# serval/kaboodle

Hardware: AMD Instinct MI355X
Metric: simulated peer-rounds/sec (whole node) + rounds to fingerprint convergence (higher is better)
Workload: dtype u8

## Files before the change

### kaboodle_amd/csrc/kb_round.h

```cpp
#pragma once
#include "kb_common.h"

namespace kb {

__global__ void k_rebase(Dev d, int32_t r) {
  const size_t total = (size_t)(d.hi - d.lo) * d.W / 16;
  const uint32_t wpr = d.W / 16;
  const int32_t E = epoch_base(r - 1);
  uint4* p = reinterpret_cast<uint4*>(d.stamp + (size_t)d.lo * d.W);
  for (size_t k = (size_t)blockIdx.x * blockDim.x + threadIdx.x; k < total; k += (size_t)gridDim.x * blockDim.x) {
    const uint4 v = p[k];
    uint32_t w[4] = {v.x, v.y, v.z, v.w};
    bool any = false;
#pragma unroll
    for (int q = 0; q < 4; ++q) {
      uint32_t x = w[q], y = 0;
#pragma unroll
      for (int t = 0; t < 4; ++t) {
        uint32_t b = (x >> (8 * t)) & 0xFF;
        if (b > ST_ANCIENT) {
          if (d.tst && b <= ST_ANCIENT + EPOCH) {
            const size_t i = d.lo + k / wpr, j = (k % wpr) * 16 + q * 4 + t;
            d.tst[i * d.W + j] = (int32_t)b - EOFF + E;
            atomicMin(d.tlb + i * (d.W >> 10) + (j >> 10), (int32_t)b - EOFF + E);
// ... 863 lines not shown
    if (threadIdx.x < 5) atomicAdd(&d.ctr[ci[threadIdx.x]], (uint32_t)(s_t[threadIdx.x] / 64));
  }
#endif
  __shared__ unsigned long long s_cnt[RP_WAVES][7];
  if (l == 0) {
    s_cnt[wv][0] = w_lost; s_cnt[wv][1] = w_removed; s_cnt[wv][2] = w_resp; s_cnt[wv][3] = w_bytes;
    s_cnt[wv][4] = a3c.x; s_cnt[wv][5] = a3c.y; s_cnt[wv][6] = a3c.z;
    if (!LDSB && w_nodes && pb.nf) path_hit(d, PATH_PHASEB_HBM);
  }
  __syncthreads();
  if (threadIdx.x < 7) {
    unsigned long long t = 0;
    for (uint32_t k = 0; k < wpb; ++k) t += s_cnt[k][threadIdx.x];
    const int idx[7] = {S_BDROP, S_RMFAILED, S_JRESP, S_ROWB, S_A3ROWS, S_A3DEEP, S_A3CHUNKS};
    if (t) slot_add(d, idx[threadIdx.x], t);
  }
}

__global__ __launch_bounds__(256) void k_probe(Dev d, uint32_t np, int32_t r, uint2* out, uint32_t* cnt, uint32_t cap) {
  const uint32_t i = d.lo + blockIdx.x * blockDim.x + threadIdx.x;
  unsigned long long lost_in = 0, sent = 0, lost_out = 0;
  if (i < d.hi && d.alive[i] && d.start_round[i] < r) {
    const bool f = faults(d, r) && d.loss_thr;
    const uint32_t n = d.n[i];
    for (uint32_t e = 0; e < np; ++e) {
      if (f) {
        const U4 w = philox(i, (uint32_t)r, ((uint32_t)P_PROBE << 24) | (e >> 2), 0, d.k0, d.k1);
        const uint32_t u = (e & 3) == 0 ? w.x : (e & 3) == 1 ? w.y : (e & 3) == 2 ? w.z : w.w;
        if (u < d.loss_thr) { lost_in++; continue; }
      }
      const int64_t o = (int64_t)n - 2;
      bool resp = o <= 0;
      if (!resp) {
        int64_t pct = 100 - o * o; if (pct < 1) pct = 1;
        const uint32_t u = philox(i, (uint32_t)r, ((uint32_t)P_RESPOND << 24) | (1u << 23) | e, 0, d.k0, d.k1).x;
        resp = (int64_t)mulhi(u, 100) < pct;
      }
      if (!resp) continue;
      sent++;
      if (f && philox(i, (uint32_t)r, ((uint32_t)P_PROBE << 24) | (1u << 23) | e, 1, d.k0, d.k1).x < d.loss_thr) { lost_out++; continue; }
      const uint32_t k = atomicAdd(cnt, 1u);
      if (k < cap) out[k] = make_uint2(i, e);
      else set_err(d, DERR_OUTBOX);
    }
  }
  const int idx[3] = {S_BDROP, S_PROBERESP, S_LOSS};
  const unsigned long long v[3] = {lost_in, sent, lost_out};
  stat_add_n(d, idx, v);
}

__device__ inline bool newbit(const unsigned long long* nm, uint32_t e) { return (nm[e >> 6] >> (e & 63)) & 1ull; }
__device__ inline uint32_t mix32(uint32_t x) {
  x ^= x >> 16; x *= 0x7feb352du; x ^= x >> 15; x *= 0x846ca68bu; x ^= x >> 16;
  return x;
}
struct Prp { uint32_t n, c, ma, mc, k[4]; };
__device__ inline Prp prp_make(uint32_t n, const U4& key) {
  const uint32_t lg = n <= 1 ? 0u : 32u - __clz(n - 1u);
  const uint32_t b = lg < 2 ? 2u : lg;
  Prp p;
  p.n = n; p.c = b / 2; p.mc = (1u << p.c) - 1u; p.ma = (1u << (b - p.c)) - 1u;
  p.k[0] = key.x; p.k[1] = key.y; p.k[2] = key.z; p.k[3] = key.w;
  return p;
}
__device__ __attribute__((always_inline)) inline uint32_t prp_pass(uint32_t x, const Prp& p) {
  uint32_t L = x >> p.c, R = x & p.mc;
#pragma unroll
  for (int k = 0; k < 4; ++k) { const uint32_t t = R; R = L ^ (mix32(R ^ p.k[k]) & ((k & 1) ? p.mc : p.ma)); L = t; }
  return (L << p.c) | R;
}
__device__ __attribute__((always_inline)) inline uint32_t prp_eval(uint32_t x, const Prp& p) {
  do { x = prp_pass(x, p); } while (x >= p.n);
  return x;
}
__device__ __attribute__((always_inline)) inline uint32_t prp_walk(uint32_t x, uint32_t n, const U4& key) {
  return prp_eval(x, prp_make(n, key));
}
__device__ inline uint32_t bm_rank(const uint32_t* S, const uint32_t* SP, uint32_t id) {
  const uint32_t blk = id >> 8, w = id >> 5;
  uint32_t r = SP[blk];
  for (uint32_t k = blk * 8; k < w; ++k) r += __popc(S[k]);
  return r + __popc(S[w] & ((1u << (id & 31)) - 1u));
}
__device__ __attribute__((always_inline)) inline uint32_t bm_block(const uint32_t* SP, uint32_t nblk, float ratio,
                                                                   uint32_t b, uint32_t* base) {
  uint32_t g = (uint32_t)((float)b * ratio);
  g = g < nblk ? g : nblk - 1;
  const uint32_t l2 = g >= 2 ? g - 2 : 0, h2 = g + 3 < nblk ? g + 3 : nblk;
  uint32_t v[6];
#pragma unroll
  for (int j = 0; j < 6; ++j) v[j] = SP[l2 + j < h2 ? l2 + j : h2];
  if (v[0] <= b && b < v[5]) {
    uint32_t c = 0, bs = v[0];
#pragma unroll
    for (int j = 1; j < 5; ++j) { const bool le = v[j] <= b; c += le; bs = le ? v[j] : bs; }
    *base = bs;
    return l2 + c;
  }
  uint32_t lo = 0, hi = nblk;
  while (hi - lo > 1) { const uint32_t mid = (lo + hi) >> 1; if (SP[mid] <= b) lo = mid; else hi = mid; }
  *base = SP[lo];
  return lo;
}
__device__ __attribute__((always_inline)) inline uint32_t block_pick(const uint4& q0, const uint4& q1, uint32_t blk,
                                                                     uint32_t rem) {
  const uint32_t p0 = __popc(q0.x), p1 = __popc(q0.y), p2 = __popc(q0.z), p3 = __popc(q0.w);
  const uint32_t p4 = __popc(q1.x), p5 = __popc(q1.y), p6 = __popc(q1.z);
  const uint32_t s01 = p0 + p1, s45 = p4 + p5, s03 = s01 + p2 + p3;
  const bool h1 = rem >= s03;
  rem -= h1 ? s03 : 0u;
  const uint32_t sa = h1 ? s45 : s01;
  const bool h2 = rem >= sa;
  rem -= h2 ? sa : 0u;
  const uint32_t pa = h1 ? (h2 ? p6 : p4) : (h2 ? p2 : p0);
  const bool h3 = rem >= pa;
  rem -= h3 ? pa : 0u;
  const uint32_t wi = (h1 ? 4u : 0u) + (h2 ? 2u : 0u) + (h3 ? 1u : 0u);
  const uint32_t xa = h1 ? (h2 ? (h3 ? q1.w : q1.z) : (h3 ? q1.y : q1.x)) : (h2 ? (h3 ? q0.w : q0.z) : (h3 ? q0.y : q0.x));
  return (blk * 8 + wi) * 32 + select_in_word(xa, rem);
}
__device__ inline uint32_t bm_select(const uint32_t* S, const uint32_t* SP, uint32_t nblk, float ratio, uint32_t b) {
  uint32_t base;
  const uint32_t lo = bm_block(SP, nblk, ratio, b, &base);
  const uint4 q0 = *reinterpret_cast<const uint4*>(S + lo * 8), q1 = *reinterpret_cast<const uint4*>(S + lo * 8 + 4);
  return block_pick(q0, q1, lo, b - base);
}
constexpr uint32_t KB_RESP_U = 2;
constexpr int RESP_U = KB_RESP_U;
constexpr int RESP_KMAX = 9;
struct JoinLds {
  const uint32_t *J, *JM;
  __device__ uint32_t min_from(uint32_t u) const { return JM[u]; }
  __device__ uint32_t at(uint32_t f) const { return J[f]; }
};
struct JoinRegs {
  uint32_t j0, j1, jmin;
  __device__ uint32_t min_from(uint32_t) const { return jmin; }
  __device__ uint32_t at(uint32_t f) const { return f < 64 ? rdl(j0, (int)f) : rdl(j1, (int)(f - 64)); }
};
template <class JA>
__device__ __attribute__((always_inline)) inline void sampled_fill(uint32_t* pay, uint32_t k_first, uint32_t stride,
                                                                   uint32_t cap, const Prp& P, const uint32_t* B,
                                                                   const uint32_t* BP, uint32_t NB, float ratio,
                                                                   const JA& J, uint32_t upto, uint32_t nnew) {
  const uint32_t jmin = J.min_from(upto);
  const uint32_t mcount = k_first < cap ? (cap - k_first + stride - 1) / stride : 0u;
  uint32_t y[RESP_KMAX];
#pragma unroll
  for (int q = 0; q < RESP_KMAX; ++q) y[q] = 0;
  if (4ull * P.n >= 3ull * ((uint64_t)(P.ma + 1) << P.c)) {
#pragma unroll
    for (int q = 0; q < RESP_KMAX; ++q) {
      const bool act = (uint32_t)q < mcount;
      if (!__ballot(act)) break;
      uint32_t x = prp_pass(k_first + stride * q, P);
      while (__ballot(act && x >= P.n)) { if (act && x >= P.n) x = prp_pass(x, P); }
      y[q] = x;
    }
  } else {
    uint32_t m = 0, x = k_first;
    while (__ballot(m < mcount)) {
      if (m < mcount) {
        x = prp_pass(x, P);
        if (x < P.n) {
#pragma unroll
          for (int q = 0; q < RESP_KMAX; ++q) if ((uint32_t)q == m) y[q] = x;
          ++m;
          x = k_first + stride * m;
        }
      }
    }
  }
#pragma unroll
  for (int q0 = 0; q0 < RESP_KMAX; q0 += RESP_U) {
    if ((uint32_t)q0 >= mcount) break;
    uint32_t blk[RESP_U], bb[RESP_U];
    uint4 b0[RESP_U], b1[RESP_U];
#pragma unroll
    for (int u = 0; u < RESP_U; ++u) {
      bb[u] = 0;
      blk[u] = q0 + u < RESP_KMAX ? bm_block(BP, NB, ratio, y[q0 + u < RESP_KMAX ? q0 + u : 0], &bb[u]) : 0u;
    }
#pragma unroll
    for (int u = 0; u < RESP_U; ++u) {
      b0[u] = *reinterpret_cast<const uint4*>(B + blk[u] * 8);
      b1[u] = *reinterpret_cast<const uint4*>(B + blk[u] * 8 + 4);
    }
#pragma unroll
    for (int u = 0; u < RESP_U; ++u) {
      const uint32_t q = q0 + u;
      if (q >= RESP_KMAX || q >= mcount) break;
      const uint32_t yq = y[q];
      uint32_t xq = block_pick(b0[u], b1[u], blk[u], yq - bb[u]);
      if (xq >= jmin) {
        uint32_t e = 0;
        while (true) {
          uint32_t c = 0;
          for (uint32_t f = upto; f < nnew; ++f) c += J.at(f) <= xq;
          if (c == e) break;
          e = c;
          xq = bm_select(B, BP, NB, ratio, yq + e);
        }
      }
      pay[k_first + stride * q] = xq;
    }
  }
}
constexpr uint32_t RESP_LDS_W = 131072;
constexpr uint32_t RESP_JCAP = 1024;
__host__ __device__ inline size_t resp_words(uint32_t NW, uint32_t NB) {
  return (2ull * NW + 2ull * (NB + 1) + 2ull * RESP_JCAP + 1 + 3) & ~3ull;
}

__device__ __attribute__((always_inline)) inline uint32_t block_prefix(const uint32_t* X, uint32_t* XP, uint32_t NB, uint32_t* s_red) {
  const uint32_t t = threadIdx.x, T = blockDim.x;
  const uint32_t per = (NB + T - 1) / T;
  uint32_t bc = 0;
  for (uint32_t k = t * per; k < (t + 1) * per && k < NB; ++k) {
    uint32_t c = 0;
    for (uint32_t w = 0; w < 8; ++w) c += __popc(X[k * 8 + w]);
    XP[k] = c; bc += c;
  }
  uint32_t ex = wave_excl(bc);
  const uint32_t wt = wave_sum(bc);
  __syncthreads();
  if (lane() == 0) s_red[t >> 6] = wt;
  __syncthreads();
  for (uint32_t w = 0; w < (t >> 6); ++w) ex += s_red[w];
  uint32_t tot = 0;
  for (uint32_t w = 0; w < T / 64; ++w) tot += s_red[w];
  for (uint32_t k = t * per; k < (t + 1) * per && k < NB; ++k) { const uint32_t c = XP[k]; XP[k] = ex; ex += c; }
  if (t == 0) XP[NB] = tot;
  __syncthreads();
  return tot;
}

constexpr uint32_t RW_JCAP = 128;
__host__ __device__ inline uint32_t rwave_head(uint32_t NB) { return ((NB + 1 > RW_JCAP ? NB + 1 : RW_JCAP) + 3) & ~3u; }
__host__ __device__ inline uint32_t rwave_words(uint32_t NW, uint32_t NB) { return rwave_head(NB) + NW; }
__device__ inline bool resp_by_wave(const Dev& d, uint32_t i, uint32_t nnew, bool on) {
  return on && d.uniform && nnew <= RW_JCAP && d.n[i] - nnew > d.capj;
}
template <bool SG>
__global__ __launch_bounds__(256) __attribute__((amdgpu_waves_per_eu(4))) void k_resp_wave(Dev d, PhaseB pb, const uint32_t* nodes, const uint32_t* nnodes_p,
                                                   OutBuf ob, int32_t r, uint32_t* rest) {
  extern __shared__ __attribute__((aligned(16))) uint32_t rw_lds[];
  const uint32_t NW = d.NWR, NB = d.W / 256;
  const uint32_t wv = threadIdx.x >> 6, l = lane(), nwv = blockDim.x >> 6;
  uint32_t* BP = rw_lds + (size_t)wv * (SG ? rwave_head(NB) : rwave_words(NW, NB));
  uint32_t* Jt = BP;
  uint32_t* S = BP + rwave_head(NB);
  const uint32_t nnodes = *nnodes_p;
  const bool small_lists = pb.JW <= 64 && pb.nj <= 128;
  const uint32_t js0 = small_lists && l < pb.nj ? pb.bjoin[l].sender : 0u;
  const uint32_t js1 = small_lists && l + 64 < pb.nj ? pb.bjoin[l + 64].sender : 0u;
  const uint32_t stride = gridDim.x * nwv;
  uint32_t it = blockIdx.x * nwv + wv;
  uint32_t inext = it < nnodes ? nodes[it] : 0u;
  for (; it < nnodes; it += stride) {
    const uint32_t i = inext;
    const unsigned long long* nm = pb.newmask + (size_t)i * pb.JW;
    const unsigned long long* rm = pb.respmask + (size_t)i * pb.JW;
    const unsigned long long nmv = small_lists && l < pb.JW ? nm[l] : 0ull;
    const unsigned long long rmv = small_lists && l < pb.JW ? rm[l] : 0ull;
    const uint32_t n_i = d.n[i], nbase_i = pb.nbase[i], poff_i = ob.poff[i], ooff_i = ob.off[i];
    inext = it + stride < nnodes ? nodes[it + stride] : 0u;
    const uint32_t* B = bits_of(d, i);
    const uint4* B4 = reinterpret_cast<const uint4*>(B);
    const bool tdbg = (d.dev & 512) != 0;
    const uint64_t tps = tdbg ? wall_clock64() : 0;
    if (!SG) stage16(reinterpret_cast<uint4*>(S), B4, NW / 4, l, 64);
    uint32_t nnew = 0;
    if (small_lists) nnew = wave_sum((uint32_t)__popcll(nmv));
    else for (uint32_t wj = 0; wj < pb.JW; ++wj) nnew += __popcll(nm[wj]);
    if (!(d.uniform && nnew <= RW_JCAP && n_i - nnew > d.capj)) {
      if (l == 0) rest[atomicAdd(&d.ctr[C_RESTN], 1u)] = i;
      wait_lds();
      __builtin_amdgcn_wave_barrier();
      continue;
    }
    if (l == 0) path_hit(d, SG ? PATH_RESP_WAVE_HBM : PATH_RESP_WAVE);
    uint64_t tp0 = tdbg ? wall_clock64() : 0, tp1 = 0, tp2 = 0;
    if (small_lists) {
      const unsigned long long w0 = ((unsigned long long)rdl((uint32_t)(nmv >> 32), 0) << 32) | rdl((uint32_t)nmv, 0);
      const unsigned long long w1 = ((unsigned long long)rdl((uint32_t)(nmv >> 32), 1) << 32) | rdl((uint32_t)nmv, 1);
      if (l < pb.nj && ((w0 >> l) & 1ull)) Jt[__popcll(w0 & ((1ull << l) - 1ull))] = js0;
      if (l + 64 < pb.nj && ((w1 >> l) & 1ull)) Jt[__popcll(w0) + __popcll(w1 & ((1ull << l) - 1ull))] = js1;
    } else {
      for (uint32_t e = l; e < pb.nj; e += 64) {
        if (!newbit(nm, e)) continue;
        uint32_t pos = __popcll(nm[e >> 6] & ((1ull << (e & 63)) - 1ull));
        for (uint32_t w2 = 0; w2 < (e >> 6); ++w2) pos += __popcll(nm[w2]);
        Jt[pos] = pb.bjoin[e].sender;
      }
    }
    wait_lds();
    __builtin_amdgcn_wave_barrier();
    const uint32_t jr0 = l < nnew ? Jt[l] : 0xFFFFFFFFu, jr1 = l + 64 < nnew ? Jt[l + 64] : 0xFFFFFFFFu;
    uint32_t sm0 = jr0, sm1 = jr1;
#pragma unroll
    for (int o = 1; o < 64; o <<= 1) {
      const uint32_t u0 = __shfl_down(sm0, o, 64), u1 = __shfl_down(sm1, o, 64);
      if (l + o < 64) { sm0 = u0 < sm0 ? u0 : sm0; sm1 = u1 < sm1 ? u1 : sm1; }
    }
    {
      const uint32_t m1 = rdl(sm1, 0);
      sm0 = m1 < sm0 ? m1 : sm0;
    }
    wait_lds();
    __builtin_amdgcn_wave_barrier();
    if (tdbg) tp1 = wall_clock64();
    const uint32_t per = (NB + 63) / 64;
    uint32_t bc = 0, last = 0;
    const uint4* S4 = reinterpret_cast<const uint4*>(SG ? B : S);
    for (uint32_t k = l * per; k < (l + 1) * per && k < NB; ++k) {
      const uint4 q0 = S4[2 * k], q1 = S4[2 * k + 1];
      const uint32_t c = __popc(q0.x) + __popc(q0.y) + __popc(q0.z) + __popc(q0.w) + __popc(q1.x) + __popc(q1.y) +
                         __popc(q1.z) + __popc(q1.w);
      BP[k] = c; bc += c;
      if (c) last = k + 1;
    }
    uint32_t ex = wave_excl(bc);
    const uint32_t nB = wave_sum(bc);
    const uint32_t nbu = wave_max(last);
    const float ratio = nB ? (float)nbu / (float)nB : 0.0f;
    for (uint32_t k = l * per; k < (l + 1) * per && k < NB; ++k) { const uint32_t c = BP[k]; BP[k] = ex; ex += c; }
    if (l == 0) BP[NB] = nB;
    wait_lds();
    __builtin_amdgcn_wave_barrier();
    uint32_t poff = poff_i, q = 0, ins_before = 0;
    if (tdbg) tp2 = wall_clock64();
    for (uint32_t wj = 0; wj < pb.JW; ++wj) {
      unsigned long long rmw, nmw;
      if (small_lists) {
        rmw = ((unsigned long long)rdl((uint32_t)(rmv >> 32), (int)wj) << 32) | rdl((uint32_t)rmv, (int)wj);
        nmw = ((unsigned long long)rdl((uint32_t)(nmv >> 32), (int)wj) << 32) | rdl((uint32_t)nmv, (int)wj);
      } else {
        rmw = rm[wj]; nmw = nm[wj];
      }
      while (rmw) {
        const uint32_t bit = (uint32_t)(__ffsll((long long)rmw) - 1);
        const uint32_t K = wj * 64 + bit;
        rmw &= rmw - 1;
        const uint32_t upto = ins_before + __popcll(nmw & ((2ull << bit) - 1ull));
        const uint32_t expect = nbase_i + upto;
        const uint32_t a = small_lists ? (K < 64 ? rdl(js0, (int)K) : rdl(js1, (int)(K - 64))) : pb.bjoin[K].sender;
        const uint32_t nk = nB - (nnew - upto), cap = d.capj;
        uint32_t* pay = ob.pay + poff;
        const Prp P = prp_make(nk, philox(i, (uint32_t)r, (uint32_t)P_TRUNC << 24, a, d.k0, d.k1));
        const uint32_t jmin = upto < 64 ? rdl(sm0, (int)upto) : upto < 128 ? rdl(sm1, (int)(upto - 64)) : 0xFFFFFFFFu;
        sampled_fill(pay, l, 64, cap, P, SG ? B : S, BP, NB, ratio, JoinRegs{jr0, jr1, jmin}, upto, nnew);
        if (l == 0) {
          Msg m; m.dest = a; m.sender = i; m.seq = q; m.kind = K_KP; m.a = cap; m.fp = 0; m.n = 0; m.off = poff;
          ob.msgs[ooff_i + q] = m;
          if (nk != expect) set_err(d, DERR_RESP);
        }
        poff += cap; q++;
      }
      ins_before += __popcll(nmw);
    }
    if (l == 0) slot_add(d, S_RESPB, 4ull * NW + 16ull * pb.JW + 4ull * pb.nj + (4ull * d.capj + 32ull) * q +
                                     (SG ? 32ull * d.capj * q : 0ull));
    if (tdbg && l == 0) {
      __builtin_amdgcn_s_waitcnt(0);
      const uint64_t tp3 = wall_clock64();
      atomicAdd(&d.ctr[C_DBG_TNODE], (uint32_t)(tp2 - tp1)); atomicAdd(&d.ctr[C_DBG_TBASE], (uint32_t)(tp1 - tp0));
      atomicAdd(&d.ctr[C_DBG_TINS], (uint32_t)(tp3 - tp2)); atomicAdd(&d.ctr[C_DBG_TSTART], 1u);
      atomicAdd(&d.ctr[C_DBG_MSGS], q); atomicAdd(&d.ctr[C_DBG_TEND], (uint32_t)(tp0 - tps));
    }
    wait_lds();
    __builtin_amdgcn_wave_barrier();
  }
}

__global__ __launch_bounds__(256) void k_resp_node(Dev d, PhaseB pb, const uint32_t* nodes, const uint32_t* nnodes_p,
                                                   OutBuf ob, int32_t r, uint32_t* gscratch, bool wave_on) {
  extern __shared__ uint32_t lds_dyn[];
  const uint32_t NW = d.NWR, NB = d.W / 256;
  uint32_t* lds = gscratch ? gscratch + (size_t)blockIdx.x * resp_words(NW, NB) : lds_dyn;
  uint32_t* B = lds;
  uint32_t* BP = B + NW;
  uint32_t* S = BP + NB + 1;
  uint32_t* SP = S + NW;
  uint32_t* J = SP + NB + 1;
  uint32_t* JM = J + RESP_JCAP;
  __shared__ uint32_t s_red[16];
  const uint32_t t = threadIdx.x, T = blockDim.x;
  const uint32_t nnodes = *nnodes_p;
  for (uint32_t it = blockIdx.x; it < nnodes; it += gridDim.x) {
    const uint32_t i = nodes[it];
    const unsigned long long* nm = pb.newmask + (size_t)i * pb.JW;
    const unsigned long long* rm = pb.respmask + (size_t)i * pb.JW;
    uint32_t nnew = 0;
    for (uint32_t wj = 0; wj < pb.JW; ++wj) nnew += __popcll(nm[wj]);
    if (resp_by_wave(d, i, nnew, wave_on)) continue;
    if (gscratch) copy16(reinterpret_cast<uint4*>(B), reinterpret_cast<const uint4*>(bits_of(d, i)), NW / 4, t, T);
    else stage16(reinterpret_cast<uint4*>(B), reinterpret_cast<const uint4*>(bits_of(d, i)), NW / 4, t, T);
    __syncthreads();
    const uint32_t nB = block_prefix(B, BP, NB, s_red);
    const bool jl = nnew <= RESP_JCAP;
    if (jl) {
      for (uint32_t e = t; e < pb.nj; e += T) {
        if (!newbit(nm, e)) continue;
        uint32_t pos = __popcll(nm[e >> 6] & ((1ull << (e & 63)) - 1ull));
        for (uint32_t w2 = 0; w2 < (e >> 6); ++w2) pos += __popcll(nm[w2]);
        J[pos] = pb.bjoin[e].sender;
      }
      __syncthreads();
      if (nnew <= T) {
        uint32_t v = t < nnew ? J[t] : 0xFFFFFFFFu;
#pragma unroll
        for (int o = 1; o < 64; o <<= 1) {
          const uint32_t u = __shfl_down(v, o, 64);
          if (lane() + o < 64) v = u < v ? u : v;
        }
        if (lane() == 0) s_red[t >> 6] = v;
        __syncthreads();
        for (uint32_t w = (t >> 6) + 1; w < T / 64; ++w) v = s_red[w] < v ? s_red[w] : v;
        if (t < nnew) JM[t] = v;
        if (t == 0) JM[nnew] = 0xFFFFFFFFu;
      } else if (t == 0) {
        uint32_t m = 0xFFFFFFFFu;
        JM[nnew] = m;
        for (uint32_t q3 = nnew; q3 > 0; --q3) { m = J[q3 - 1] < m ? J[q3 - 1] : m; JM[q3 - 1] = m; }
      }
    }
    __syncthreads();
    uint32_t poff = ob.poff[i], q = 0, ins_before = 0;
    for (uint32_t wj = 0; wj < pb.JW; ++wj) {
      unsigned long long rmw = rm[wj];
      const unsigned long long nmw = nm[wj];
      while (rmw) {
        const uint32_t bit = (uint32_t)(__ffsll((long long)rmw) - 1);
        const uint32_t K = wj * 64 + bit;
        rmw &= rmw - 1;
        const uint32_t upto = ins_before + __popcll(nmw & ((2ull << bit) - 1ull));
        const uint32_t expect = pb.nbase[i] + upto;
        const uint32_t a = pb.bjoin[K].sender;
        const uint32_t nk = nB - (nnew - upto);
        const bool sample = d.uniform && nk > d.capj;
        const uint32_t cap = sample ? d.capj : nk;
        uint32_t* pay = ob.pay + poff;
        if (sample) {
          const Prp P = prp_make(nk, philox(i, (uint32_t)r, (uint32_t)P_TRUNC << 24, a, d.k0, d.k1));
          const float ratio = nB ? (float)NB / (float)nB : 0.0f;
          if (jl) {
            sampled_fill(pay, t, T, cap, P, B, BP, NB, ratio, JoinLds{J, JM}, upto, nnew);
          } else {
            for (uint32_t k = t; k < cap; k += T) {
              const uint32_t y = prp_eval(k, P);
              uint32_t e = 0, x;
              while (true) {
                x = bm_select(B, BP, NB, ratio, y + e);
                uint32_t c = 0;
                for (uint32_t f = K + 1; f < pb.nj; ++f)
                  if (newbit(nm, f)) c += pb.bjoin[f].sender <= x;
                if (c == e) break;
                e = c;
              }
              pay[k] = x;
            }
          }
        } else {
          for (uint32_t k = t; k < NW; k += T) S[k] = B[k];
          __syncthreads();
          for (uint32_t f = K + 1 + t; f < pb.nj; f += T)
            if (newbit(nm, f)) { const uint32_t x = pb.bjoin[f].sender; atomicAnd(&S[x >> 5], ~(1u << (x & 31))); }
          __syncthreads();
          block_prefix(S, SP, NB, s_red);
          for (uint32_t w = t; w < NW; w += T) {
            uint32_t x = S[w];
            if (!x) continue;
            uint32_t pos = bm_rank(S, SP, w * 32);
            while (x) { const uint32_t b = __ffs(x) - 1; x &= x - 1; pay[pos++] = w * 32 + b; }
          }
        }
        if (t == 0) {
          Msg m; m.dest = a; m.sender = i; m.seq = q; m.kind = K_KP; m.a = cap; m.fp = 0; m.n = 0; m.off = poff;
          ob.msgs[ob.off[i] + q] = m;
          if (nk != expect) set_err(d, DERR_RESP);
          if (gscratch) path_hit(d, sample ? PATH_RESP_SCRATCH_SAMPLED : PATH_RESP_SCRATCH_FULL);
        }
        poff += cap; q++;
        __syncthreads();
      }
      ins_before += __popcll(nmw);
    }
  }
}

}
```

### kaboodle_amd/csrc/kb_sim.hip

```cpp
#include <hip/hip_runtime.h>
#include <hip/hip_ext.h>
#include <stdint.h>
#include <stdio.h>
#include <string.h>
#include <stdlib.h>
#include <string>
#include <vector>
#include <array>
#include <algorithm>
#include <atomic>
#include <thread>
#include "kb_common.h"
#include "kb_wire.h"
#include "kb_round.h"
#include "kb_tick.h"
#include "kb_waves.h"
#include "kb_xfer.h"
#include "kb_sparse.h"

using namespace kb;

enum KId : int {
  KI_REBASE, KI_EVENTS, KI_CHURN_LEAVE, KI_CHURN_JOIN, KI_ALIVE_BITS, KI_TRUEFP_PART, KI_TRUEFP_FIN, KI_LOG_MARK,
  KI_LAT_MARK, KI_BFAIL_PREP, KI_ROWPASS, KI_LAT_SWEEP, KI_SCAN_TILES, KI_SCAN_APPLY, KI_SET_CAP, KI_RESP_WAVE,
// ... 274 lines not shown
  hipEvent_t ev_fork[4] = {nullptr, nullptr, nullptr, nullptr}, ev_join[4] = {nullptr, nullptr, nullptr, nullptr};
  uint32_t C, W, S;
  uint32_t lo, hi, R;
  int rank, world;
  Xfer* xf;
  bool in_group;
  std::vector<void*> allocs;
  int32_t round;
  bool probed = false;
  std::vector<uint8_t> h_ident, h_idlen;
  std::vector<uint8_t> h_pend; std::vector<int16_t> h_pendlen;
  std::vector<uint8_t> h_moved;
  std::vector<uint8_t> h_idset;
  std::vector<uint8_t> h_ext;
  size_t n_ext = 0;
  std::vector<XRec> inj; std::vector<uint32_t> inj_ids;
  std::vector<uint32_t> inj_join;
  XRec* d_inj = nullptr; uint32_t* d_inj_ids = nullptr; size_t d_inj_cap = 0, d_inj_ids_cap = 0;
  std::vector<kb_unicast> xq; std::vector<uint32_t> xq_ids;
  std::vector<Event> events;
  uint32_t* rpack = nullptr; uint32_t* rpack_in = nullptr;
  std::vector<kb_wire_addr> probe_q, probes;
  std::vector<kb_probe_response> presp;
  uint2* d_presp = nullptr; uint32_t* d_presp_n = nullptr; size_t presp_cap = 0;
  OutBuf ob[2];
  WaveCtl wc;
  uint32_t msg_cap, pay_cap;
  BCast* bfail; BCast* bjoin;
  BCast* bfail_loc; BCast* bjoin_loc;
  uint32_t nf, nj;
  uint32_t ucap = 0;
  uint64_t xbytes_cross = 0, xbytes_all = 0;
  BcastSlots bs;
  uint32_t* join_off; uint32_t* fail_off;
  uint32_t* scan_tot; uint32_t* scan_tiles;
  unsigned long long* newmask; unsigned long long* respmask; size_t mask_words;
  unsigned long long* newmask_base; unsigned long long* respmask_base;
  uint32_t* nresp; uint32_t* paysum; uint32_t* nbase; uint32_t* resp_off;
  uint32_t* resp_nodes; uint32_t* bf_gid; uint8_t* bf_dep;
  uint32_t* slow;
  uint32_t* defer = nullptr;
  uint32_t* w0ctr = nullptr;
  uint16_t* lat_col;
  uint32_t* fnamed;
  uint32_t* resp_scratch; size_t resp_scratch_words;
  RowOut ro;
  Event* d_events; uint32_t events_cap;
  XState xs;
  uint32_t* xall; unsigned long long* xstats;
  std::vector<uint32_t> h_xall;
  Msg* rmsg; uint32_t* rpay; uint8_t* rstatus; uint32_t* rinbox; uint32_t* rkp;
  size_t rmsg_cap, rpay_cap;
  double round_ms;
  uint32_t* rr = nullptr;
  uint64_t round_launches, bj_total, bf_total;
  struct KRec { int16_t kid, wave; hipEvent_t a, b; };
  int prof_level = 1;
  bool capturing = false;
  int cur_wave = -1;
  std::vector<hipEvent_t> ev_free;
  std::vector<KRec> krec;
  double k_ms[NKI] = {};
  double k_wms[NKI][KB_WAVE_SLOTS] = {};
  uint64_t k_n[NKI] = {};
  uint64_t k_bytes0[NSTAT] = {};
  uint64_t host_syncs = 0;
  uint32_t ncu = 256;
  uint32_t* cs_buf = nullptr;
  uint32_t* rc_buf = nullptr;
  void* rc_pairs = nullptr; size_t rc_pairs_cap = 0;
  void* fc_buf = nullptr; size_t fc_cap = 0;
  double census_ms[CM_N] = {};
  bool debug_waves = false;
  size_t lds_per_cu = 65536;
  std::vector<kb_sim*> shards;
  LocalHub* hub;
  std::vector<uint32_t> watch_node, watch_fp;
  std::vector<uint32_t*> watch_snap;
  uint32_t* ev_out = nullptr;
  uint32_t* h_pin = nullptr;
  uint32_t* d_pin = nullptr;
  uint32_t pin_seq = 0;
  uint64_t occ_key = ~0ull; int occ_val = 0;
  bool graph_on = false;
  hipGraph_t wave_graph = nullptr; hipGraphExec_t wave_exec = nullptr;
  uint64_t buf_gen = 0, wave_gen = ~0ull;
  uint32_t* lc_buf = nullptr;
  double sn_ms = 0;
};

template <class T> static hipError_t talloc(kb_sim* s, T** p, size_t n) {
  hipError_t e = dalloc(p, n);
  if (e == hipSuccess) s->allocs.push_back((void*)*p);
  return e;
}
template <class T> static T* bias(T* base, size_t per_row, uint32_t lo) {
  return reinterpret_cast<T*>(reinterpret_cast<uintptr_t>(base) - sizeof(T) * per_row * lo);
}
template <class T> static hipError_t ralloc(kb_sim* s, T** p, size_t per_row) {
  T* base = nullptr;
  hipError_t e = talloc(s, &base, per_row * s->R);
  *p = bias(base, per_row, s->lo);
  return e;
}
template <class T> static T* L(const kb_sim* s, T* p) { return p + s->lo; }

static void prof_events(kb_sim* s, int kid, hipEvent_t* a, hipEvent_t* b) {
  *a = *b = nullptr;
  if (s->capturing || s->prof_level <= 0 || (s->prof_level == 1 && (kbytes_stat(kid) < 0 || kid == KI_PROC))) return;
  hipEvent_t e[2];
  for (int k = 0; k < 2; ++k) {
    if (!s->ev_free.empty()) { e[k] = s->ev_free.back(); s->ev_free.pop_back(); }
    else if (hipEventCreate(&e[k]) != hipSuccess) { if (k) s->ev_free.push_back(e[0]); return; }
  }
  *a = e[0]; *b = e[1];
  const int w = s->cur_wave < 0 ? -1 : (s->cur_wave < KB_WAVE_SLOTS ? s->cur_wave : KB_WAVE_SLOTS - 1);
  s->krec.push_back(kb_sim::KRec{(int16_t)kid, (int16_t)w, e[0], e[1]});
}
template <typename F, typename... Args>
static void klaunch_on(kb_sim* s, hipStream_t stream, int kid, F kern, dim3 grid, dim3 block, uint32_t lds, Args... args) {
  hipEvent_t a, b;
  prof_events(s, kid, &a, &b);
  hipExtLaunchKernelGGL(kern, grid, block, lds, stream, a, b, 0, args...);
}
template <typename F, typename... Args>
static void klaunch(kb_sim* s, int kid, F kern, dim3 grid, dim3 block, uint32_t lds, Args... args) {
  klaunch_on(s, s->st, kid, kern, grid, block, lds, args...);
}
static void side_fork(kb_sim* s, int k) { (void)hipEventRecord(s->ev_fork[k], s->st); (void)hipStreamWaitEvent(s->st2, s->ev_fork[k], 0); }
static void side_done(kb_sim* s, int k) { (void)hipEventRecord(s->ev_join[k], s->st2); }
static void side_join(kb_sim* s, int k) { (void)hipStreamWaitEvent(s->st, s->ev_join[k], 0); }
static void prof_resolve(kb_sim* s, size_t n) {
  n = std::min(n, s->krec.size());
  for (size_t k = 0; k < n; ++k) {
    const kb_sim::KRec& q = s->krec[k];
    float ms = 0;
    hipError_t e = hipEventElapsedTime(&ms, q.a, q.b);
    if (e == hipErrorNotReady) {
      (void)hipGetLastError();
      (void)hipEventSynchronize(q.b);
      e = hipEventElapsedTime(&ms, q.a, q.b);
    }
    if (e == hipSuccess) {
      if (q.kid == NKI) { s->round_ms += ms; s->round_launches++; }
      else {
        s->k_ms[q.kid] += ms; s->k_n[q.kid]++;
        if (q.wave >= 0) s->k_wms[q.kid][q.wave] += ms;
      }
    }
    s->ev_free.push_back(q.a); s->ev_free.push_back(q.b);
  }
  s->krec.erase(s->krec.begin(), s->krec.begin() + n);
}

static ScanArgs scan_args(kb_sim* s, uint32_t n, uint32_t* totals) {
  ScanArgs a; memset(&a, 0, sizeof a); a.n = n; a.totals = totals;
  a.tiles = s->scan_tiles; a.ntiles = (n + 1023) / 1024; return a;
}
static void launch_scan(kb_sim* s, const ScanArgs& a) {
  if (!a.n) return;
  klaunch(s, KI_SCAN_TILES, k_scan_tiles, dim3(a.ntiles), dim3(1024), 0, a);
  klaunch(s, KI_SCAN_APPLY, k_scan_apply, dim3(a.ntiles), dim3(1024), 0, a);
}

extern "C" void kb_config_default(kb_config* c) {
  memset(c, 0, sizeof *c);
// ... 819 lines not shown
    }
  }
  side_fork(s, 0);
  klaunch_on(s, s->st2, KI_ALIVE_BITS, k_alive_bits, dim3((d.NWR + tb - 1) / tb), dim3(tb), 0, d);
  klaunch_on(s, s->st2, KI_TRUEFP_PART, k_truefp_part, dim3(TRUEFP_G), dim3(256), 0, d, d.tfpart);
  klaunch_on(s, s->st2, KI_TRUEFP_FIN, k_truefp_fin, dim3(1), dim3(64), 0, d, d.tfpart);
  side_done(s, 0);
  if (lat_fail) {
    klaunch_on(s, s->st2, KI_LAT_SWEEP, k_lat_sweep, dim3((lat_stride(R) / 8 + 255) / 256, std::min<uint32_t>(s->nf, 16384)), dim3(256), 0, d,
            (const BCast*)s->bfail, (const uint32_t*)s->bf_gid, s->nf, s->fnamed);
    side_done(s, 1);
  }
  s->probes.swap(s->probe_q);
  s->probe_q.clear();
  const uint32_t np = (uint32_t)s->probes.size();
  if (np) {
    const size_t need = (size_t)np * R;
    if (need > s->presp_cap) {
      if (s->d_presp) (void)hipFree(s->d_presp);
      s->d_presp = nullptr;
      HIPCHK(hipMalloc(&s->d_presp, sizeof(uint2) * need));
      s->presp_cap = need;
    }
    if (!s->d_presp_n) HIPCHK(hipMalloc(&s->d_presp_n, 4));
    HIPCHK(hipMemsetAsync(s->d_presp_n, 0, 4, st));
    klaunch(s, KI_PROBE, k_probe, dim3(gnode), dim3(tb), 0, d, np, r, s->d_presp, s->d_presp_n, (uint32_t)s->presp_cap);
  }
  const uint32_t ninj = (uint32_t)s->inj.size();
  bool inj_pay = false;
  if (ninj) {
    if (ninj > s->d_inj_cap) {
      if (s->d_inj) (void)hipFree(s->d_inj);
      s->d_inj_cap = 2 * ninj;
      HIPCHK(hipMalloc(&s->d_inj, sizeof(XRec) * s->d_inj_cap));
    }
    if (s->inj_ids.size() > s->d_inj_ids_cap || !s->d_inj_ids) {
      if (s->d_inj_ids) (void)hipFree(s->d_inj_ids);
      s->d_inj_ids_cap = 2 * s->inj_ids.size() + 16;
      HIPCHK(hipMalloc(&s->d_inj_ids, 4 * s->d_inj_ids_cap));
    }
    HIPCHK(hipMemcpyAsync(s->d_inj, s->inj.data(), sizeof(XRec) * ninj, hipMemcpyHostToDevice, st));
    if (!s->inj_ids.empty()) {
      HIPCHK(hipMemcpyAsync(s->d_inj_ids, s->inj_ids.data(), 4 * s->inj_ids.size(), hipMemcpyHostToDevice, st));
      inj_pay = true;
    }
    klaunch(s, KI_EVENTS, k_inject_prep, dim3(1), dim3(64), 0, d, (const XRec*)s->d_inj, ninj, s->paysum);
  }
  {
    ScanArgs a = scan_args(s, R, s->scan_tot);
    a.narr = 3;
    a.in[0] = L(s, s->nresp); a.out[0] = L(s, s->resp_off);
    a.in[1] = L(s, s->paysum); a.out[1] = L(s, o0.poff);
    a.in[2] = L(s, s->nresp); a.out[2] = L(s, o0.off); a.addc[2] = TICK_MAX;
    a.list = s->resp_nodes; a.list_base = s->lo;
    launch_scan(s, a);
  }
  const bool need_tot = (have_b && s->nj) || inj_pay;
  klaunch(s, KI_SET_CAP, k_set_cap, dim3(gnode), dim3(tb), 0, d, s->nresp, o0.cap, o0.cnt, s->scan_tot, s->d_pin, need_tot ? ++s->pin_seq : 0u);
  if (need_tot) {
    const uint32_t* tot = s->h_pin;
    { const int rc = wait_pin(s, s->pin_seq); if (rc) return rc; }
    const uint32_t pay_tot = tot[1], msg_tot = tot[2], resp_nodes = tot[4];
    if (msg_tot > o0.msg_cap || pay_tot > o0.pay_cap) {
      const int rc = grow_wave0(s, msg_tot, pay_tot);
      if (rc) return rc;
    }
    if (s->n_ext) { const int rc = size_exports(s, msg_tot, pay_tot); if (rc) return rc; }
    if (resp_nodes) {
      const uint32_t grid = std::min<uint32_t>(resp_nodes, 4096);
      const size_t words = resp_words(d.NWR, s->W / 256);
      uint32_t* scratch = nullptr;
      size_t lds = 4 * words;
      const bool resp_hbm = s->W > RESP_LDS_W || (d.dbg & KB_DBG_RESP_HBM);
      if (resp_hbm) {
        if (s->resp_scratch_words < words * grid) {
          if (s->resp_scratch) (void)hipFree(s->resp_scratch);
          HIPCHK(hipMalloc(&s->resp_scratch, 4 * words * grid));
          s->resp_scratch_words = words * grid;
        }
        scratch = s->resp_scratch;
        lds = 0;
      }
      const size_t wlds = 16ull * rwave_words(d.NWR, s->W / 256);
      const size_t hlds = 4ull * rwave_head(s->W / 256);
      const bool full_on = wlds <= 65536 && !(d.dbg & (KB_DBG_RESP_HBM | KB_DBG_RESP_WAVE_HBM));
      const uint32_t hwaves = (uint32_t)std::min<size_t>(4, 65536 / hlds);
      const bool head_on = !full_on && hwaves >= 1 && !(d.dbg & KB_DBG_RESP_HBM);
      const bool wave_on = full_on || head_on;
      if (s->debug_waves) HIPCHK(hipMemsetAsync(d.ctr + C_DBG_INS, 0, 52, st));
      if (full_on) {
        klaunch(s, KI_RESP_WAVE, k_resp_wave<false>, dim3(std::min<uint32_t>((resp_nodes + 3) / 4, 4096)), dim3(256), (uint32_t)wlds, d,
                pb, (const uint32_t*)s->resp_nodes, (const uint32_t*)(s->scan_tot + 4), o0, r, s->slow);
      } else if (head_on) {
        klaunch(s, KI_RESP_WAVE, k_resp_wave<true>, dim3(std::min<uint32_t>((resp_nodes + hwaves - 1) / hwaves, 4096)),
                dim3(64 * hwaves), (uint32_t)(hwaves * hlds), d, pb, (const uint32_t*)s->resp_nodes,
                (const uint32_t*)(s->scan_tot + 4), o0, r, s->slow);
      }
      klaunch(s, KI_RESP_NODE, k_resp_node, dim3(wave_on ? std::min<uint32_t>(grid, 2 * s->ncu) : grid), dim3(256), (uint32_t)lds, d, pb,
              (const uint32_t*)(wave_on ? s->slow : s->resp_nodes), (const uint32_t*)(wave_on ? d.ctr + C_RESTN : s->scan_tot + 4),
              o0, r, scratch, wave_on);
      if (s->debug_waves && (d.dev & 512)) {
        uint32_t dbg[13];
        HIPCHK(hipMemcpyAsync(dbg, d.ctr + C_DBG_INS, 52, hipMemcpyDeviceToHost, st));
        HIPCHK(hipStreamSynchronize(st));
        fprintf(stderr, "[kb] round %d k_resp_wave: responders %u, responses %u: row staging %.1f us, joiners %.1f, prefix %.1f, "
                "fills %.1f (sums over waves)\n", r, dbg[10], dbg[12], dbg[11] * 0.01, dbg[8] * 0.01, dbg[6] * 0.01, dbg[9] * 0.01);
      }
    }
  }
  if (lat_fail) side_join(s, 1);
  klaunch(s, KI_TICK_SCAN, k_tick_scan, dim3(gnode), dim3(tb), 0, d, s->bs, r, s->slow);
  klaunch(s, KI_TICK_PRE, k_tick_pre, dim3(std::min<uint32_t>(gwave, 1024)), dim3(256), 0, d, o0, s->bs, r, s->slow);
  if (d.tst) {
    side_fork(s, 2);
    const uint32_t kpl = a3_kpl(s->W, d.dbg);
    if (kpl == 2) klaunch_on(s, s->st2, KI_A3_EXACT, k_a3_exact<2>, dim3((R + 3) / 4), dim3(256), 0, d, s->ro.part, r);
    else if (kpl) klaunch_on(s, s->st2, KI_A3_EXACT, k_a3_exact<A3X_KPL>, dim3((R + 3) / 4), dim3(256), 0, d, s->ro.part, r);
    else klaunch_on(s, s->st2, KI_A3_EXACT, k_a3_exact<0>, dim3((R + 3) / 4), dim3(256), 0, d, s->ro.part, r);
    side_done(s, 2);
  }
  if (d.uniform) klaunch(s, KI_FOLD, k_fold, dim3(((R + 63) / 64 + 3) / 4 * s->S), dim3(256), 0, d, FoldArgs{s->S});
  if (d.uniform) klaunch(s, KI_FP_ROWS, k_fp_rows, dim3((FP_LANES * R + tb - 1) / tb), dim3(tb), 0, d);
  side_join(s, 0);
  if (d.tst) side_join(s, 2);
  klaunch(s, KI_TICK_POST, k_tick_post, dim3(gnode), dim3(tb), 0, d, s->ro, o0, r);
  if (ninj) {
    klaunch(s, KI_EVENTS, k_inject, dim3(1), dim3(64), 0, d, o0, (const XRec*)s->d_inj, ninj, (const uint32_t*)s->d_inj_ids);
    s->inj.clear(); s->inj_ids.clear();
  }
  {
    ScanArgs a = scan_args(s, R, s->scan_tot);
    a.narr = 2;
    a.in[0] = L(s, s->bs.join); a.out[0] = L(s, s->join_off);
    a.in[1] = L(s, s->bs.nfail); a.out[1] = L(s, s->fail_off);
    launch_scan(s, a);
  }
  klaunch(s, KI_BCAST_WRITE, k_bcast_write, dim3(gnode), dim3(tb), 0, d, s->bs, (const uint32_t*)s->join_off,
          (const uint32_t*)s->fail_off, s->xf ? s->bjoin_loc : s->bjoin, s->xf ? s->bfail_loc : s->bfail);
  if (!s->xf && !s->debug_waves && s->graph_on) {
    if (!s->wave_exec || s->wave_gen != s->buf_gen) {
      if (s->wave_exec) { (void)hipGraphExecDestroy(s->wave_exec); s->wave_exec = nullptr; }
      if (s->wave_graph) { (void)hipGraphDestroy(s->wave_graph); s->wave_graph = nullptr; }
      HIPCHK(hipStreamBeginCapture(st, hipStreamCaptureModeThreadLocal));
      s->capturing = true;
      const int rc = launch_waves(s, -1);
      s->capturing = false;
      hipGraph_t g = nullptr;
      const hipError_t e = hipStreamEndCapture(st, &g);
      if (rc) { if (g) (void)hipGraphDestroy(g); return rc; }
      HIPCHK(e);
      s->wave_graph = g;
      HIPCHK(hipGraphInstantiate(&s->wave_exec, g, nullptr, nullptr, 0));
      s->wave_gen = s->buf_gen;
    }
    HIPCHK(hipGraphLaunch(s->wave_exec, st));
  } else {
    const int rc = launch_waves(s, r);
    if (rc) return rc;
  }
  if (s->xf && !s->xf->allreduce_sum_u32(d.ctr + C_AGREE, 1, st)) { seterr(s->xf->error()); return KB_IO_ERROR; }
  klaunch(s, KI_ROUND_END, k_round_end, dim3(1), dim3(1), 0, d, r, (const uint32_t*)s->scan_tot, s->d_pin,
          s->xf ? 0u : ++s->pin_seq, s->rr);
  (void)hipEventRecord(er[1], st);
  s->krec.push_back(kb_sim::KRec{(int16_t)NKI, (int16_t)-1, er[0], er[1]});
  prof_resolve(s, krec0);
  uint32_t err = 0;
  if (s->xf) {
    const int rc = gather_broadcasts(s, &err);
    if (rc) return rc;
  } else {
    const int rc = wait_pin(s, s->pin_seq);
    if (rc) return rc;
    s->nj = s->h_pin[0]; s->nf = s->h_pin[1]; err = s->h_pin[2];
  }
  s->bj_total += s->nj; s->bf_total += s->nf;
  if (s->n_ext) {
    uint32_t c[2];
    HIPCHK(hipMemcpy(c, d.ctr + C_XREC, 8, hipMemcpyDeviceToHost));
    const uint32_t nrec = std::min(c[0], d.xrec_cap), nid = std::min(c[1], d.xids_cap);
// ... 640 lines not shown
```

Baseline: 12.65 million.

## Replace ratio-guess block search with rank-sampled lookup table for bitmap select

Builds a sampled rank table (one entry per 256 set bits) alongside the block prefix sums in LDS, so select finds its block with one table lookup plus a short forward scan. This replaces the float-ratio guess, its six-entry window and the binary-search fallback. It adds LDS for the table and per-block writes during the prefix pass. The head-only wave variant coarsens the table stride, and the waves-per-workgroup rule changes, to protect occupancy.

```diff
diff --git a/kaboodle_amd/csrc/kb_round.h b/kaboodle_amd/csrc/kb_round.h
--- a/kaboodle_amd/csrc/kb_round.h
+++ b/kaboodle_amd/csrc/kb_round.h
@@ -969,25 +969,26 @@
   for (uint32_t k = blk * 8; k < w; ++k) r += __popc(S[k]);
   return r + __popc(S[w] & ((1u << (id & 31)) - 1u));
 }
-__device__ __attribute__((always_inline)) inline uint32_t bm_block(const uint32_t* SP, uint32_t nblk, float ratio,
-                                                                   uint32_t b, uint32_t* base) {
-  uint32_t g = (uint32_t)((float)b * ratio);
-  g = g < nblk ? g : nblk - 1;
-  const uint32_t l2 = g >= 2 ? g - 2 : 0, h2 = g + 3 < nblk ? g + 3 : nblk;
-  uint32_t v[6];
-#pragma unroll
-  for (int j = 0; j < 6; ++j) v[j] = SP[l2 + j < h2 ? l2 + j : h2];
-  if (v[0] <= b && b < v[5]) {
-    uint32_t c = 0, bs = v[0];
-#pragma unroll
-    for (int j = 1; j < 5; ++j) { const bool le = v[j] <= b; c += le; bs = le ? v[j] : bs; }
-    *base = bs;
-    return l2 + c;
-  }
-  uint32_t lo = 0, hi = nblk;
-  while (hi - lo > 1) { const uint32_t mid = (lo + hi) >> 1; if (SP[mid] <= b) lo = mid; else hi = mid; }
-  *base = SP[lo];
-  return lo;
+constexpr uint32_t RT_RS = 8;
+__host__ __device__ inline uint32_t rt_len(uint32_t NB, uint32_t rs) { return (NB >> (rs - 8)) + 1; }
+__host__ __device__ inline uint32_t rt_words(uint32_t NB, uint32_t rs) { return (rt_len(NB, rs) + 3) & ~3u; }
+struct RankIdx { const uint32_t *BP, *RT; uint32_t NB, rs; };
+__device__ __attribute__((always_inline)) inline void rt_own(uint32_t* RT, uint32_t rs, uint32_t k, uint32_t lo, uint32_t hi) {
+  const uint32_t q = (lo + (1u << rs) - 1u) >> rs;
+  if ((q << rs) < hi) RT[q] = k;
+}
+__device__ __attribute__((always_inline)) inline void rt_tail(uint32_t* RT, uint32_t rs, uint32_t NB, uint32_t total, uint32_t t,
+                                                              uint32_t T) {
+  for (uint32_t q = ((total + (1u << rs) - 1u) >> rs) + t; q < rt_len(NB, rs); q += T) RT[q] = NB - 1;
+}
+__device__ __attribute__((always_inline)) inline uint32_t rank_block(const RankIdx& X, uint32_t b, uint32_t* base) {
+  uint32_t blk = X.RT[b >> X.rs];
+  uint32_t lo = X.BP[blk], n1 = X.BP[blk + 1];
+  const uint32_t n2 = X.BP[blk + 2 < X.NB ? blk + 2 : X.NB];
+  if (b >= n1 && blk + 1 < X.NB) { ++blk; lo = n1; n1 = n2; }
+  while (b >= n1 && blk + 1 < X.NB) { ++blk; lo = n1; n1 = X.BP[blk + 1]; }
+  *base = lo;
+  return blk;
 }
 __device__ __attribute__((always_inline)) inline uint32_t block_pick(const uint4& q0, const uint4& q1, uint32_t blk,
                                                                      uint32_t rem) {
@@ -1006,9 +1007,9 @@
   const uint32_t xa = h1 ? (h2 ? (h3 ? q1.w : q1.z) : (h3 ? q1.y : q1.x)) : (h2 ? (h3 ? q0.w : q0.z) : (h3 ? q0.y : q0.x));
   return (blk * 8 + wi) * 32 + select_in_word(xa, rem);
 }
-__device__ inline uint32_t bm_select(const uint32_t* S, const uint32_t* SP, uint32_t nblk, float ratio, uint32_t b) {
+__device__ inline uint32_t bm_select(const uint32_t* S, const RankIdx& X, uint32_t b) {
   uint32_t base;
-  const uint32_t lo = bm_block(SP, nblk, ratio, b, &base);
+  const uint32_t lo = rank_block(X, b, &base);
   const uint4 q0 = *reinterpret_cast<const uint4*>(S + lo * 8), q1 = *reinterpret_cast<const uint4*>(S + lo * 8 + 4);
   return block_pick(q0, q1, lo, b - base);
 }
@@ -1028,8 +1029,8 @@
 template <class JA>
 __device__ __attribute__((always_inline)) inline void sampled_fill(uint32_t* pay, uint32_t k_first, uint32_t stride,
                                                                    uint32_t cap, const Prp& P, const uint32_t* B,
-                                                                   const uint32_t* BP, uint32_t NB, float ratio,
-                                                                   const JA& J, uint32_t upto, uint32_t nnew) {
+                                                                   const RankIdx& X, const JA& J, uint32_t upto,
+                                                                   uint32_t nnew) {
   const uint32_t jmin = J.min_from(upto);
   const uint32_t mcount = k_first < cap ? (cap - k_first + stride - 1) / stride : 0u;
   uint32_t y[RESP_KMAX];
@@ -1066,7 +1067,7 @@
 #pragma unroll
     for (int u = 0; u < RESP_U; ++u) {
       bb[u] = 0;
-      blk[u] = q0 + u < RESP_KMAX ? bm_block(BP, NB, ratio, y[q0 + u < RESP_KMAX ? q0 + u : 0], &bb[u]) : 0u;
+      blk[u] = q0 + u < RESP_KMAX ? rank_block(X, y[q0 + u < RESP_KMAX ? q0 + u : 0], &bb[u]) : 0u;
     }
 #pragma unroll
     for (int u = 0; u < RESP_U; ++u) {
@@ -1086,7 +1087,7 @@
           for (uint32_t f = upto; f < nnew; ++f) c += J.at(f) <= xq;
           if (c == e) break;
           e = c;
-          xq = bm_select(B, BP, NB, ratio, yq + e);
+          xq = bm_select(B, X, yq + e);
         }
       }
       pay[k_first + stride * q] = xq;
@@ -1096,10 +1097,11 @@
 constexpr uint32_t RESP_LDS_W = 131072;
 constexpr uint32_t RESP_JCAP = 1024;
 __host__ __device__ inline size_t resp_words(uint32_t NW, uint32_t NB) {
-  return (2ull * NW + 2ull * (NB + 1) + 2ull * RESP_JCAP + 1 + 3) & ~3ull;
-}
-
-__device__ __attribute__((always_inline)) inline uint32_t block_prefix(const uint32_t* X, uint32_t* XP, uint32_t NB, uint32_t* s_red) {
+  return ((2ull * NW + 2ull * (NB + 1) + 2ull * RESP_JCAP + 1 + 3) & ~3ull) + rt_words(NB, RT_RS);
+}
+
+__device__ __attribute__((always_inline)) inline uint32_t block_prefix(const uint32_t* X, uint32_t* XP, uint32_t NB, uint32_t* s_red,
+                                                                       uint32_t* RT = nullptr) {
   const uint32_t t = threadIdx.x, T = blockDim.x;
   const uint32_t per = (NB + T - 1) / T;
   uint32_t bc = 0;
@@ -1116,27 +1118,42 @@
   for (uint32_t w = 0; w < (t >> 6); ++w) ex += s_red[w];
   uint32_t tot = 0;
   for (uint32_t w = 0; w < T / 64; ++w) tot += s_red[w];
-  for (uint32_t k = t * per; k < (t + 1) * per && k < NB; ++k) { const uint32_t c = XP[k]; XP[k] = ex; ex += c; }
+  for (uint32_t k = t * per; k < (t + 1) * per && k < NB; ++k) {
+    const uint32_t c = XP[k];
+    XP[k] = ex;
+    if (RT) rt_own(RT, RT_RS, k, ex, ex + c);
+    ex += c;
+  }
   if (t == 0) XP[NB] = tot;
+  if (RT) rt_tail(RT, RT_RS, NB, tot, t, T);
   __syncthreads();
   return tot;
 }
 
 constexpr uint32_t RW_JCAP = 128;
-__host__ __device__ inline uint32_t rwave_head(uint32_t NB) { return ((NB + 1 > RW_JCAP ? NB + 1 : RW_JCAP) + 3) & ~3u; }
-__host__ __device__ inline uint32_t rwave_words(uint32_t NW, uint32_t NB) { return rwave_head(NB) + NW; }
+__host__ __device__ inline uint32_t rwave_bp(uint32_t NB) { return ((NB + 1 > RW_JCAP ? NB + 1 : RW_JCAP) + 3) & ~3u; }
+__host__ __device__ inline uint32_t rwave_head(uint32_t NB, uint32_t rs) { return rwave_bp(NB) + rt_words(NB, rs); }
+__host__ __device__ inline uint32_t rwave_words(uint32_t NW, uint32_t NB) { return rwave_head(NB, RT_RS) + NW; }
+__host__ inline uint32_t resp_head_waves(uint32_t head_words) { return head_words <= 4096 ? 4u : 16384u / head_words; }
+__host__ inline uint32_t resp_head_rs(uint32_t NB) {
+  uint32_t rs = RT_RS;
+  while (rs < 16 && resp_head_waves(rwave_head(NB, rs)) < resp_head_waves(rwave_bp(NB))) ++rs;
+  return rs;
+}
 __device__ inline bool resp_by_wave(const Dev& d, uint32_t i, uint32_t nnew, bool on) {
   return on && d.uniform && nnew <= RW_JCAP && d.n[i] - nnew > d.capj;
 }
 template <bool SG>
 __global__ __launch_bounds__(256) __attribute__((amdgpu_waves_per_eu(4))) void k_resp_wave(Dev d, PhaseB pb, const uint32_t* nodes, const uint32_t* nnodes_p,
-                                                   OutBuf ob, int32_t r, uint32_t* rest) {
+                                                   OutBuf ob, int32_t r, uint32_t* rest, uint32_t rs_head) {
   extern __shared__ __attribute__((aligned(16))) uint32_t rw_lds[];
   const uint32_t NW = d.NWR, NB = d.W / 256;
   const uint32_t wv = threadIdx.x >> 6, l = lane(), nwv = blockDim.x >> 6;
-  uint32_t* BP = rw_lds + (size_t)wv * (SG ? rwave_head(NB) : rwave_words(NW, NB));
+  const uint32_t rs = SG ? rs_head : RT_RS;
+  uint32_t* BP = rw_lds + (size_t)wv * (SG ? rwave_head(NB, rs) : rwave_words(NW, NB));
   uint32_t* Jt = BP;
-  uint32_t* S = BP + rwave_head(NB);
+  uint32_t* RT = BP + rwave_bp(NB);
+  uint32_t* S = BP + rwave_head(NB, rs);
   const uint32_t nnodes = *nnodes_p;
   const bool small_lists = pb.JW <= 64 && pb.nj <= 128;
   const uint32_t js0 = small_lists && l < pb.nj ? pb.bjoin[l].sender : 0u;
@@ -1198,21 +1215,25 @@
     __builtin_amdgcn_wave_barrier();
     if (tdbg) tp1 = wall_clock64();
     const uint32_t per = (NB + 63) / 64;
-    uint32_t bc = 0, last = 0;
+    uint32_t bc = 0;
     const uint4* S4 = reinterpret_cast<const uint4*>(SG ? B : S);
     for (uint32_t k = l * per; k < (l + 1) * per && k < NB; ++k) {
       const uint4 q0 = S4[2 * k], q1 = S4[2 * k + 1];
       const uint32_t c = __popc(q0.x) + __popc(q0.y) + __popc(q0.z) + __popc(q0.w) + __popc(q1.x) + __popc(q1.y) +
                          __popc(q1.z) + __popc(q1.w);
       BP[k] = c; bc += c;
-      if (c) last = k + 1;
     }
     uint32_t ex = wave_excl(bc);
     const uint32_t nB = wave_sum(bc);
-    const uint32_t nbu = wave_max(last);
-    const float ratio = nB ? (float)nbu / (float)nB : 0.0f;
-    for (uint32_t k = l * per; k < (l + 1) * per && k < NB; ++k) { const uint32_t c = BP[k]; BP[k] = ex; ex += c; }
+    for (uint32_t k = l * per; k < (l + 1) * per && k < NB; ++k) {
+      const uint32_t c = BP[k];
+      BP[k] = ex;
+      rt_own(RT, rs, k, ex, ex + c);
+      ex += c;
+    }
     if (l == 0) BP[NB] = nB;
+    rt_tail(RT, rs, NB, nB, l, 64);
+    const RankIdx X{BP, RT, NB, rs};
     wait_lds();
     __builtin_amdgcn_wave_barrier();
     uint32_t poff = poff_i, q = 0, ins_before = 0;
@@ -1236,7 +1257,7 @@
         uint32_t* pay = ob.pay + poff;
         const Prp P = prp_make(nk, philox(i, (uint32_t)r, (uint32_t)P_TRUNC << 24, a, d.k0, d.k1));
         const uint32_t jmin = upto < 64 ? rdl(sm0, (int)upto) : upto < 128 ? rdl(sm1, (int)(upto - 64)) : 0xFFFFFFFFu;
-        sampled_fill(pay, l, 64, cap, P, SG ? B : S, BP, NB, ratio, JoinRegs{jr0, jr1, jmin}, upto, nnew);
+        sampled_fill(pay, l, 64, cap, P, SG ? B : S, X, JoinRegs{jr0, jr1, jmin}, upto, nnew);
         if (l == 0) {
           Msg m; m.dest = a; m.sender = i; m.seq = q; m.kind = K_KP; m.a = cap; m.fp = 0; m.n = 0; m.off = poff;
           ob.msgs[ooff_i + q] = m;
@@ -1271,6 +1292,8 @@
   uint32_t* SP = S + NW;
   uint32_t* J = SP + NB + 1;
   uint32_t* JM = J + RESP_JCAP;
+  uint32_t* RT = lds + resp_words(NW, NB) - rt_words(NB, RT_RS);
+  const RankIdx X{BP, RT, NB, RT_RS};
   __shared__ uint32_t s_red[16];
   const uint32_t t = threadIdx.x, T = blockDim.x;
   const uint32_t nnodes = *nnodes_p;
@@ -1284,7 +1307,7 @@
     if (gscratch) copy16(reinterpret_cast<uint4*>(B), reinterpret_cast<const uint4*>(bits_of(d, i)), NW / 4, t, T);
     else stage16(reinterpret_cast<uint4*>(B), reinterpret_cast<const uint4*>(bits_of(d, i)), NW / 4, t, T);
     __syncthreads();
-    const uint32_t nB = block_prefix(B, BP, NB, s_red);
+    const uint32_t nB = block_prefix(B, BP, NB, s_red, RT);
     const bool jl = nnew <= RESP_JCAP;
     if (jl) {
       for (uint32_t e = t; e < pb.nj; e += T) {
@@ -1330,15 +1353,14 @@
         uint32_t* pay = ob.pay + poff;
         if (sample) {
           const Prp P = prp_make(nk, philox(i, (uint32_t)r, (uint32_t)P_TRUNC << 24, a, d.k0, d.k1));
-          const float ratio = nB ? (float)NB / (float)nB : 0.0f;
           if (jl) {
-            sampled_fill(pay, t, T, cap, P, B, BP, NB, ratio, JoinLds{J, JM}, upto, nnew);
+            sampled_fill(pay, t, T, cap, P, B, X, JoinLds{J, JM}, upto, nnew);
           } else {
             for (uint32_t k = t; k < cap; k += T) {
               const uint32_t y = prp_eval(k, P);
               uint32_t e = 0, x;
               while (true) {
-                x = bm_select(B, BP, NB, ratio, y + e);
+                x = bm_select(B, X, y + e);
                 uint32_t c = 0;
                 for (uint32_t f = K + 1; f < pb.nj; ++f)
                   if (newbit(nm, f)) c += pb.bjoin[f].sender <= x;
diff --git a/kaboodle_amd/csrc/kb_sim.hip b/kaboodle_amd/csrc/kb_sim.hip
--- a/kaboodle_amd/csrc/kb_sim.hip
+++ b/kaboodle_amd/csrc/kb_sim.hip
@@ -380,6 +380,7 @@
   uint32_t* d_pin = nullptr;
   uint32_t pin_seq = 0;
   uint64_t occ_key = ~0ull; int occ_val = 0;
+  bool resp_occ_said = false;
   bool graph_on = false;
   hipGraph_t wave_graph = nullptr; hipGraphExec_t wave_exec = nullptr;
   uint64_t buf_gen = 0, wave_gen = ~0ull;
@@ -1365,19 +1366,29 @@
         lds = 0;
       }
       const size_t wlds = 16ull * rwave_words(d.NWR, s->W / 256);
-      const size_t hlds = 4ull * rwave_head(s->W / 256);
+      const uint32_t hrs = resp_head_rs(s->W / 256);
+      const size_t hlds = 4ull * rwave_head(s->W / 256, hrs);
       const bool full_on = wlds <= 65536 && !(d.dbg & (KB_DBG_RESP_HBM | KB_DBG_RESP_WAVE_HBM));
-      const uint32_t hwaves = (uint32_t)std::min<size_t>(4, 65536 / hlds);
+      const uint32_t hwaves = resp_head_waves((uint32_t)(hlds / 4));
       const bool head_on = !full_on && hwaves >= 1 && !(d.dbg & KB_DBG_RESP_HBM);
       const bool wave_on = full_on || head_on;
       if (s->debug_waves) HIPCHK(hipMemsetAsync(d.ctr + C_DBG_INS, 0, 52, st));
+      if (s->debug_waves && wave_on && !s->resp_occ_said) {
+        int occ = 0;
+        const void* rk = full_on ? reinterpret_cast<const void*>(&k_resp_wave<false>) : reinterpret_cast<const void*>(&k_resp_wave<true>);
+        const size_t l = full_on ? wlds : hwaves * hlds;
+        (void)hipOccupancyMaxActiveBlocksPerMultiprocessor(&occ, rk, full_on ? 256 : (int)(64 * hwaves), l);
+        fprintf(stderr, "[kb] k_resp_wave<%s>: %u waves/workgroup, %zu B LDS (rank stride %u), %d workgroups/CU\n",
+                full_on ? "false" : "true", full_on ? 4u : hwaves, l, full_on ? RT_RS : hrs, occ);
+        s->resp_occ_said = true;
+      }
       if (full_on) {
         klaunch(s, KI_RESP_WAVE, k_resp_wave<false>, dim3(std::min<uint32_t>((resp_nodes + 3) / 4, 4096)), dim3(256), (uint32_t)wlds, d,
-                pb, (const uint32_t*)s->resp_nodes, (const uint32_t*)(s->scan_tot + 4), o0, r, s->slow);
+                pb, (const uint32_t*)s->resp_nodes, (const uint32_t*)(s->scan_tot + 4), o0, r, s->slow, RT_RS);
       } else if (head_on) {
         klaunch(s, KI_RESP_WAVE, k_resp_wave<true>, dim3(std::min<uint32_t>((resp_nodes + hwaves - 1) / hwaves, 4096)),
                 dim3(64 * hwaves), (uint32_t)(hwaves * hlds), d, pb, (const uint32_t*)s->resp_nodes,
-                (const uint32_t*)(s->scan_tot + 4), o0, r, s->slow);
+                (const uint32_t*)(s->scan_tot + 4), o0, r, s->slow, hrs);
       }
       klaunch(s, KI_RESP_NODE, k_resp_node, dim3(wave_on ? std::min<uint32_t>(grid, 2 * s->ncu) : grid), dim3(256), (uint32_t)lds, d, pb,
               (const uint32_t*)(wave_on ? s->slow : s->resp_nodes), (const uint32_t*)(wave_on ? d.ctr + C_RESTN : s->scan_tot + 4),
```

Result: slower. 12.51 million (-1.1%).
